# BolinLai/CSTS

Hardware: AMD Instinct MI355X
Metric: clips/sec training (fwd+bwd) CSTS-Ego4D 16x256^2 bf16 (higher is better)
Workload: dtype bf16; 1 GPU; CSTS_Ego4D_Gaze_Forecast.yaml train step (fwd + KLDiv + 0.05*EgoNCE + bwd + clip + AdamW), 16x256^2 video + 24 kHz STFT audio, b=4/GPU; mode=train, global_batch=4, frames=16, crop=256, parallelism=dp1, step=hip_graph, hip_graph=True, rccl_ranks=1

## Files before the change

### csts_amd/csrc/attention.hip

```cpp
#include <type_traits>
#include <utility>
#include "common.h"

#ifndef CSTS_ATTN_PART
#define CSTS_ATTN_PART 0
#endif
#ifndef CSTS_DKV_DEPTH
#define CSTS_DKV_DEPTH 4
#endif
#ifndef CSTS_DKV_SWZ
#define CSTS_DKV_SWZ 0
#endif

#ifdef CSTS_ATTN_STAMPS
#if CSTS_ATTN_PART == 1
__device__ unsigned long long g_attn_stamps[4096];
#else
static __device__ unsigned long long g_attn_stamps[4096];
#endif
#define AT_STAMP() do { if (stamp_on && nstamp < 4000) g_attn_stamps[nstamp++] = (unsigned long long)__builtin_amdgcn_s_memtime(); } while (0)
#if CSTS_ATTN_PART == 1
extern "C" int csts_debug_attn_stamps(unsigned long long* dst_host) {
  return (int)hipMemcpyFromSymbol(dst_host, HIP_SYMBOL(g_attn_stamps), sizeof(unsigned long long) * 4096);
}
// ... 1465 lines not shown
  CSTS_REQUIRE(a->O && a->LSE && aligned16(a->O) && strides_ok(a->o_strides, a->dtype), "bad output");
  AttnP p; fill(a, p);
  dim3 grid((unsigned)cdiv(a->Nq, 128), a->H, a->B);
  CSTS_REQUIRE(attn_dispatch(K_FWD, a, p, grid, stream), "hipFuncSetAttribute(MaxDynamicSharedMemorySize) failed on this device");
  CSTS_LAUNCH_CHECK();
  return 0;
}

extern "C" size_t csts_attn_bwd_workspace(const csts_attn_args* a) {
  if (!a) return 0;
  int nsplit, q_chunk;
  dkv_plan(a, nsplit, q_chunk);
  return nsplit > 1 ? (size_t)2 * nsplit * a->B * a->H * a->Nk * a->head_dim * sizeof(float) : 16;
}

extern "C" int csts_attn_bwd(const csts_attn_args* a, void* workspace, size_t ws_bytes, hipStream_t stream) {
  ATTN_COMMON_CHECKS(a);
  CSTS_REQUIRE(a->O && a->LSE && a->dO && a->delta && a->dQ && a->dK && a->dV, "null backward operand");
  CSTS_REQUIRE(aligned16(a->dO) && aligned16(a->dQ) && aligned16(a->dK) && aligned16(a->dV), "alignment");
  CSTS_REQUIRE(strides_ok(a->do_strides, a->dtype) && strides_ok(a->dq_strides, a->dtype) &&
                   strides_ok(a->dk_strides, a->dtype) && strides_ok(a->dv_strides, a->dtype) &&
                   strides_ok(a->o_strides, a->dtype), "strides must keep 16-byte row alignment");
  AttnP p; fill(a, p);
  if (fused_bwd_ok(a)) {
    dkv_plan(a, p.nsplit, p.q_chunk);
    if (p.nsplit > 1) {
      CSTS_REQUIRE(workspace != nullptr && ws_bytes >= csts_attn_bwd_workspace(a), "workspace too small");
      p.ws = reinterpret_cast<float*>(workspace);
    }
    hipLaunchKernelGGL((attn_bwd_fused_kernel<96>), dim3((unsigned)p.nsplit, (unsigned)(a->B * a->H)), dim3(256), 0, stream, p);
    CSTS_LAUNCH_CHECK();
    if (p.nsplit > 1) {
      const int64_t total = (int64_t)2 * a->B * a->H * a->Nk * a->head_dim / 8;
      hipLaunchKernelGGL(attn_dkv_reduce_kernel, dim3((unsigned)std::min<int64_t>(cdiv(total, 256), 4096)), dim3(256), 0,
                         stream, p, a->head_dim);
      CSTS_LAUNCH_CHECK();
    }
    return 0;
  }
  {
    dim3 grid((unsigned)cdiv(a->Nq, 128), a->H, a->B);
    CSTS_REQUIRE(attn_dispatch(K_DQ, a, p, grid, stream), "hipFuncSetAttribute(MaxDynamicSharedMemorySize) failed on this device");
    CSTS_LAUNCH_CHECK();
  }
  {
    dkv_plan(a, p.nsplit, p.q_chunk);
    if (p.nsplit > 1) {
      CSTS_REQUIRE(workspace != nullptr && ws_bytes >= csts_attn_bwd_workspace(a), "workspace too small");
      p.ws = reinterpret_cast<float*>(workspace);
    }
    dim3 grid((unsigned)cdiv(a->Nk, 128), p.nsplit, a->B * a->H);
    CSTS_REQUIRE(attn_dispatch(K_DKV, a, p, grid, stream), "hipFuncSetAttribute(MaxDynamicSharedMemorySize) failed on this device");
    CSTS_LAUNCH_CHECK();
    if (p.nsplit > 1) {
      const int64_t total = (int64_t)2 * a->B * a->H * a->Nk * a->head_dim / 8;
      hipLaunchKernelGGL(attn_dkv_reduce_kernel, dim3((unsigned)std::min<int64_t>(cdiv(total, 256), 4096)), dim3(256), 0,
                         stream, p, a->head_dim);
      CSTS_LAUNCH_CHECK();
    }
  }
  return 0;
}

extern "C" int csts_attn_probs(const csts_attn_args* a, float* probs, hipStream_t stream) {
  ATTN_COMMON_CHECKS(a);
  CSTS_REQUIRE(a->LSE && probs, "null pointer");
  AttnP p; fill(a, p);
  const int64_t total = (int64_t)a->B * a->H * a->Nq * a->Nk;
  hipLaunchKernelGGL(attn_probs_kernel, dim3((unsigned)std::min<int64_t>(cdiv(total, 256), 4096)), dim3(256), 0, stream, p,
                     a->head_dim, probs);
  CSTS_LAUNCH_CHECK();
  return 0;
}
#else
}
bool csts_attn_dkv_fast_launch(const csts_attn::AttnP& p, dim3 grid, hipStream_t stream) {
// ... 7 lines not shown
```

### csts_amd/csrc/common.h

```cpp
#pragma once
#include <hip/hip_runtime.h>
#include <stdint.h>
#include <stddef.h>
#include <string>

#include "../../include/csts_hip.h"

#ifdef CSTS_HALF_F16
typedef _Float16 bf16;
typedef _Float16 bf16x8 __attribute__((ext_vector_type(8)));
typedef _Float16 bf16x4 __attribute__((ext_vector_type(4)));
typedef _Float16 bf16x2 __attribute__((ext_vector_type(2)));
#define CSTS_MFMA16 __builtin_amdgcn_mfma_f32_32x32x16_f16
#else
typedef __bf16 bf16;
typedef __bf16 bf16x8 __attribute__((ext_vector_type(8)));
typedef __bf16 bf16x4 __attribute__((ext_vector_type(4)));
typedef __bf16 bf16x2 __attribute__((ext_vector_type(2)));
#define CSTS_MFMA16 __builtin_amdgcn_mfma_f32_32x32x16_bf16
#endif
typedef short s16x4 __attribute__((ext_vector_type(4)));
typedef float f32x16 __attribute__((ext_vector_type(16)));
typedef float f32x4 __attribute__((ext_vector_type(4)));
typedef float f32x2 __attribute__((ext_vector_type(2)));
// ... 149 lines not shown
}
__device__ __forceinline__ float gelu_fast(float x) {
  const float t = x * 0.70710678118654752f, ax = fabsf(t);
  const float e = __expf(-ax * ax);
  const float er = copysignf(erf_poly_times_exp(ax, e), x);
  return 0.5f * x * (1.0f + er);
}
__device__ __forceinline__ float dgelu_fast(float x) {
  const float t = x * 0.70710678118654752f, ax = fabsf(t);
  const float e = __expf(-ax * ax);
  const float er = copysignf(erf_poly_times_exp(ax, e), x);
  return 0.5f * (1.0f + er) + x * 0.39894228040143268f * e;
}

int csts_reduce_rows_launch(const float* ws, float* out, int64_t nrows, int64_t ncols, float scale, hipStream_t s);
```

### csts_amd/csrc/norm.hip

```cpp
#include "common.h"

namespace {

constexpr int MAXV = 12;
constexpr int LN_BWD_WAVES = 8;

template <bool F32> __device__ __forceinline__ float ldt(const void* p, int64_t i) {
  if constexpr (F32) return reinterpret_cast<const float*>(p)[i];
  else return h16_lo((unsigned)reinterpret_cast<const unsigned short*>(p)[i]);
}
template <bool F32> __device__ __forceinline__ void stt(void* p, int64_t i, float v) {
  if constexpr (F32) reinterpret_cast<float*>(p)[i] = v;
  else reinterpret_cast<bf16*>(p)[i] = (bf16)v;
}

struct FwdAdd {
  const void* addend = nullptr;
  void* sum = nullptr;
};
template <int NV, int R, bool XF32, bool YF32>
__global__ __launch_bounds__(256) void ln_fwd_kernel(const void* __restrict__ x, const float* __restrict__ gamma,
                                                     const float* __restrict__ beta, void* __restrict__ y,
                                                     float* __restrict__ mean, float* __restrict__ rstd, int64_t rows,
                                                     int C, float eps, FwdAdd fa) {
// ... 252 lines not shown
        if (sub == 0) {
          if (mean) mean[row] = mu;
          if (rstd) rstd[row] = rs;
        }
      }
    }
  }
}

#ifndef CSTS_LN_BWD_R
#define CSTS_LN_BWD_R 1
#endif
#ifndef CSTS_LN_BWD_MINW
#define CSTS_LN_BWD_MINW 1
#endif
template <int GL, int NCH, int R, bool DYF32, bool XF32>
__global__ __launch_bounds__(512, CSTS_LN_BWD_MINW) void ln_bwd_vec_kernel(const void* __restrict__ dy, const void* __restrict__ x,
                                                         const float* __restrict__ gamma, const float* __restrict__ mean,
                                                         const float* __restrict__ rstd, void* __restrict__ dx,
                                                         const void* __restrict__ addend, float* __restrict__ ws, int64_t rows,
                                                         int C, const float* __restrict__ gamma1, Copy16 dx16) {
  extern __shared__ __attribute__((aligned(16))) float red[];
  const int64_t ro = (int64_t)blockIdx.y * rows;
  if (blockIdx.y == 1) gamma = gamma1;
  ws += (int64_t)blockIdx.y * gridDim.x * 2 * C;
  const int sub = threadIdx.x % GL, gib = threadIdx.x / GL;
  constexpr int GPB = 512 / GL;
  const int64_t grp = xcd_block(blockIdx.x, gridDim.x) * GPB + gib, ngrp = (int64_t)gridDim.x * GPB;
  int c0[NCH];
  bool act[NCH];
  float gm[NCH][8], dg[NCH][8], db[NCH][8];
#pragma unroll
  for (int i = 0; i < NCH; ++i) {
    const int c = (sub + GL * i) * 8;
    act[i] = c < C;
    c0[i] = min(c, C - 8);
    ld8t<true>(gamma, c0[i], gm[i]);
#pragma unroll
    for (int j = 0; j < 8; ++j) { dg[i][j] = 0.f; db[i][j] = 0.f; }
  }
  const float invC = 1.f / C;
  for (int64_t row0 = grp * R; row0 < rows; row0 += ngrp * R) {
    float d[R][NCH][8], xv[R][NCH][8], ad[R][NCH][8], mu[R], rs[R];
#pragma unroll
    for (int r = 0; r < R; ++r) {
      const int64_t row = ro + min(row0 + r, rows - 1);
      mu[r] = mean[row];
      rs[r] = rstd[row];
#pragma unroll
      for (int i = 0; i < NCH; ++i) {
        ld8t<DYF32>(dy, row * C + c0[i], d[r][i]);
        if (dx16.dy2) {
          float d2[8];
          ld8t<DYF32>(dx16.dy2, row * C + c0[i], d2);
#pragma unroll
          for (int j = 0; j < 8; ++j) d[r][i][j] += d2[j];
        }
        ld8t<XF32>(x, row * C + c0[i], xv[r][i]);
        if (addend) ld8t<XF32>(addend, row * C + c0[i], ad[r][i]);
        else {
#pragma unroll
          for (int j = 0; j < 8; ++j) ad[r][i][j] = 0.f;
        }
      }
    }
#pragma unroll
// ... 181 lines not shown
  else if (xf) hipLaunchKernelGGL((ln_bwd_kernel<NV, R, false, true>), grid, dim3(64 * LN_BWD_WAVES), sh, st, dy, x, g, mean, rstd, dx, addend, ws, rows, C, g1, dx16);
  else hipLaunchKernelGGL((ln_bwd_kernel<NV, R, false, false>), grid, dim3(64 * LN_BWD_WAVES), sh, st, dy, x, g, mean, rstd, dx, addend, ws, rows, C, g1, dx16);
}
template <int GL, int NCH, int R>
static void ln_fwd_vec_launch(bool xf, bool yf, dim3 grid, hipStream_t st, const void* x, const float* g, const float* b, void* y,
                              float* mean, float* rstd, int64_t rows, int C, float eps, FwdAdd fa) {
  if (xf && yf) hipLaunchKernelGGL((ln_fwd_vec_kernel<GL, NCH, R, true, true>), grid, dim3(256), 0, st, x, g, b, y, mean, rstd, rows, C, eps, fa);
  else if (xf) hipLaunchKernelGGL((ln_fwd_vec_kernel<GL, NCH, R, true, false>), grid, dim3(256), 0, st, x, g, b, y, mean, rstd, rows, C, eps, fa);
  else if (yf) hipLaunchKernelGGL((ln_fwd_vec_kernel<GL, NCH, R, false, true>), grid, dim3(256), 0, st, x, g, b, y, mean, rstd, rows, C, eps, fa);
  else hipLaunchKernelGGL((ln_fwd_vec_kernel<GL, NCH, R, false, false>), grid, dim3(256), 0, st, x, g, b, y, mean, rstd, rows, C, eps, fa);
}
template <int GL, int NCH, int R>
static void ln_bwd_vec_launch(bool df, bool xf, dim3 grid, size_t sh, hipStream_t st, const void* dy, const void* x, const float* g,
                              const float* mean, const float* rstd, void* dx, const void* addend, float* ws, int64_t rows, int C,
                              const float* g1, Copy16 dx16) {
  if (df && xf) hipLaunchKernelGGL((ln_bwd_vec_kernel<GL, NCH, R, true, true>), grid, dim3(512), sh, st, dy, x, g, mean, rstd, dx, addend, ws, rows, C, g1, dx16);
  else if (df) hipLaunchKernelGGL((ln_bwd_vec_kernel<GL, NCH, R, true, false>), grid, dim3(512), sh, st, dy, x, g, mean, rstd, dx, addend, ws, rows, C, g1, dx16);
  else if (xf) hipLaunchKernelGGL((ln_bwd_vec_kernel<GL, NCH, R, false, true>), grid, dim3(512), sh, st, dy, x, g, mean, rstd, dx, addend, ws, rows, C, g1, dx16);
  else hipLaunchKernelGGL((ln_bwd_vec_kernel<GL, NCH, R, false, false>), grid, dim3(512), sh, st, dy, x, g, mean, rstd, dx, addend, ws, rows, C, g1, dx16);
}
static bool ln_vec_ok(int C, std::initializer_list<const void*> ptrs) {
  if (C % 8 != 0 || C < 8 || C > 1024) return false;
  for (const void* q : ptrs)
    if (q != nullptr && !aligned16(q)) return false;
  return true;
}
static int ln_group_lanes(int C) { return C <= 128 ? 16 : (C <= 256 ? 32 : 64); }
#ifndef CSTS_LN_FWD_R
#define CSTS_LN_FWD_R 2
#endif
static int64_t ln_fwd_vec_blocks(int64_t rows, int C) { return std::min<int64_t>(cdiv(rows * ln_group_lanes(C), 256 * (C <= 512 ? CSTS_LN_FWD_R : 2)), 4096); }
static bool ln_bwd_vec(bool df, bool xf, dim3 grid, hipStream_t st, const void* dy, const void* x, const float* g, const float* mean,
                       const float* rstd, void* dx, const void* addend, float* ws, int64_t rows, int C, const float* g1, Copy16 dx16) {
  const size_t sh = (size_t)(512 / ln_group_lanes(C)) * 2 * C * sizeof(float);
// ... 120 lines not shown
    }
    return 0;
  }
  if (C <= 128) ln_bwd_launch<2, 4>(df, xf, grid, sh, stream, dy, x, gamma0, mean, rstd, dx, nullptr, ws, rows, C, gamma1);
  else if (C <= 192) ln_bwd_launch<3, 4>(df, xf, grid, sh, stream, dy, x, gamma0, mean, rstd, dx, nullptr, ws, rows, C, gamma1);
  else if (C <= 384) ln_bwd_launch<6, 2>(df, xf, grid, sh, stream, dy, x, gamma0, mean, rstd, dx, nullptr, ws, rows, C, gamma1);
  else ln_bwd_launch<12, 1>(df, xf, grid, sh, stream, dy, x, gamma0, mean, rstd, dx, nullptr, ws, rows, C, gamma1);
  CSTS_LAUNCH_CHECK();
  if (dgb0 != nullptr) {
    csts_reduce_rows_launch(ws, dgb0, nb, 2 * C, 1.f, stream);
    csts_reduce_rows_launch(ws + nb * 2 * C, dgb1, nb, 2 * C, 1.f, stream);
    CSTS_LAUNCH_CHECK();
  }
  return 0;
}
```

### csts_amd/csrc/stencil.hip

```cpp
#include "common.h"
#include <algorithm>
#include <cstdlib>
#include <cstring>
#include <vector>

namespace {

struct Geom {
  int B, C, HD;
  int Tf, Hf, Wf;
  int Tc, Hc, Wc;
  int st, sh, sw;
  int64_t f_bs, f_ts;
  int64_t c_bs, c_ts;
};

constexpr int VEC = 4;

__device__ __forceinline__ void ld4(const void* p, int dt, int64_t i, float (&o)[4]) {
  if (dt == CSTS_F32) {
    float4 a = *reinterpret_cast<const float4*>(reinterpret_cast<const float*>(p) + i);
    o[0] = a.x; o[1] = a.y; o[2] = a.z; o[3] = a.w;
  } else {
    bf16x4 a = *reinterpret_cast<const bf16x4*>(reinterpret_cast<const bf16*>(p) + i);
// ... 25 lines not shown
  return dt == CSTS_F32 ? (const void*)(reinterpret_cast<const float*>(p) + off) : (const void*)(reinterpret_cast<const bf16*>(p) + off);
}
__device__ __forceinline__ void* batch_ptr(void* p, int dt, int64_t off) {
  return dt == CSTS_F32 ? (void*)(reinterpret_cast<float*>(p) + off) : (void*)(reinterpret_cast<bf16*>(p) + off);
}

__device__ __forceinline__ void stage_weights(const float* __restrict__ w, float* wl, int HD) {
  const int nthr = blockDim.x * blockDim.y, tid = threadIdx.y * blockDim.x + threadIdx.x;
  for (int i = tid; i < HD * 27; i += nthr) {
    const int k = i / HD, c = i - k * HD;
    wl[i] = w[c * 27 + k];
  }
  __syncthreads();
}

struct FastDiv { unsigned m; int sh; int d; };
__device__ __forceinline__ int fdiv(int n, const FastDiv& f) { return (int)(((unsigned long long)(unsigned)n * f.m) >> f.sh); }
struct RowGeom {
  Geom g;
  int lt, lh, lw;
  FastDiv dNc, dHc, dWc;
  FastDiv dNf, dHf, dWf;
  FastDiv dN2, dH2, dW2;
  FastDiv dC4, dC8, dHD, dHeads;
};
__device__ __forceinline__ void decompf(int bt, const FastDiv& dN, const FastDiv& dH, const FastDiv& dW, int& b, int& t, int& h, int& w) {
  b = fdiv(bt, dN);
  int o = bt - b * dN.d;
  const int q = fdiv(o, dW);
  w = o - q * dW.d;
  t = fdiv(q, dH);
  h = q - t * dH.d;
// ... 1069 lines not shown
  return on;
}
bool fast_row(int row_tokens, int C, int64_t rows, FastRow& fr) {
  fr.cq = C / VEC;
  fr.wq = row_tokens * fr.cq;
  fr.inv_cq = 1.f / (float)fr.cq;
  return resample_fast_on() && C % VEC == 0 && fr.cq <= 256 && fr.wq <= 16384 && rows <= 65535 * (int64_t)1 && rows > 0;
}

int grid_for(int64_t total) { return (int)std::min<int64_t>(cdiv(total, 256), 256 * 32); }
int grid_for_staged(int64_t total) { return (int)std::min<int64_t>(cdiv(total, 256), 256 * 4); }

int ilog2(int v) { if (v <= 0 || (v & (v - 1)) != 0) return -1; int l = 0; while ((1 << l) < v) ++l; return l; }
bool pow2(int v) { return v > 0 && (v & (v - 1)) == 0; }

FastDiv fast_div(int d) {
  FastDiv f; f.d = d;
  if (d <= 1) { f.m = 1; f.sh = 0; return f; }
  int sft = 0;
  while ((1LL << sft) < d) ++sft;
  const unsigned long long num = 1ULL << (31 + sft);
  f.m = (unsigned)((num + d - 1) / d);
  f.sh = 31 + sft;
  return f;
}
int fill_geom(const csts_dwconv_geom* a, RowGeom& rg) {
  Geom& g = rg.g;
  g.B = a->B; g.C = a->C; g.HD = a->HD;
  g.Tf = a->Tf; g.Hf = a->Hf; g.Wf = a->Wf; g.Tc = a->Tc; g.Hc = a->Hc; g.Wc = a->Wc;
  g.st = a->st; g.sh = a->sh; g.sw = a->sw;
  g.f_bs = a->fine_batch_stride; g.f_ts = a->fine_token_stride;
  g.c_bs = a->coarse_batch_stride; g.c_ts = a->coarse_token_stride;
  rg.lt = ilog2(a->st); rg.lh = ilog2(a->sh); rg.lw = ilog2(a->sw);
  rg.dNc = fast_div(a->Tc * a->Hc * a->Wc); rg.dHc = fast_div(a->Hc); rg.dWc = fast_div(a->Wc);
  rg.dNf = fast_div(a->Tf * a->Hf * a->Wf); rg.dHf = fast_div(a->Hf); rg.dWf = fast_div(a->Wf);
  rg.dN2 = fast_div(std::max(1, a->Tf * (a->Hf / 2) * (a->Wf / 2))); rg.dH2 = fast_div(std::max(1, a->Hf / 2)); rg.dW2 = fast_div(std::max(1, a->Wf / 2));
  rg.dC4 = fast_div(std::max(1, a->C / 4)); rg.dC8 = fast_div(std::max(1, a->C / 8)); rg.dHD = fast_div(a->HD); rg.dHeads = fast_div(a->C / a->HD);
  return 0;
}

// ... 353 lines not shown
```

### csts_amd/lib.py

```python
from __future__ import annotations

import ctypes as C
import os

_lib = None


class CstsError(RuntimeError):
    pass


_HERE = os.path.dirname(os.path.abspath(__file__))
LIB_PATH = os.environ.get("CSTS_HIP_LIB") or os.path.join(_HERE, "libcsts_hip.so")
HALF = os.environ.get("CSTS_HALF", "bf16")
_PATHS = {"bf16": LIB_PATH, "fp16": os.environ.get("CSTS_HIP_LIB_F16") or os.path.join(_HERE, "libcsts_hip_f16.so")}


def set_half(kind: str):
    global HALF, LIB_PATH
    if kind not in _PATHS:
        raise ValueError(f"16-bit type must be 'bf16' or 'fp16', got {kind!r}")
    if _lib is not None and kind != HALF:
        raise CstsError(f"this process already runs the {HALF} kernel library; the {kind} build is a different shared object "
                        "(one 16-bit activation type per process: start a new process for the other mode)")
    HALF = kind
    LIB_PATH = _PATHS[kind]


def half_dtype():
    import torch
    return torch.float16 if HALF == "fp16" else torch.bfloat16


ABI_VERSION = 11
F32, BF16 = 0, 1
GEMM_NT, GEMM_NN, GEMM_TN = 0, 1, 2
EPI_NONE, EPI_GELU, EPI_DGELU = 0, 1, 2
MASK_NONE, MASK_SPATIAL = 0, 1
GAZE_DECODE_MAX_HW = 8192
AUDIO_PIXEL_MAX_SIDE, AUDIO_PIXEL_MAX_HW = 128, 4096

vp = C.c_void_p
i64 = C.c_int64
sz = C.c_size_t


class GemmArgs(C.Structure):
    _fields_ = [("layout", C.c_int),
                ("A", vp), ("a_dt", C.c_int), ("lda", i64),
# ... 36 lines not shown
    _fields_ = [("B", C.c_int), ("C", C.c_int),
                ("Ti", C.c_int), ("Hi", C.c_int), ("Wi", C.c_int),
                ("To", C.c_int), ("Ho", C.c_int), ("Wo", C.c_int),
                ("st", C.c_int), ("sh", C.c_int), ("sw", C.c_int)]


class AttnArgs(C.Structure):
    _fields_ = [("Q", vp), ("K", vp), ("V", vp), ("O", vp), ("LSE", vp),
                ("dO", vp), ("delta", vp), ("dQ", vp), ("dK", vp), ("dV", vp),
                ("dtype", C.c_int), ("B", C.c_int), ("H", C.c_int), ("Nq", C.c_int), ("Nk", C.c_int),
                ("head_dim", C.c_int),
                ("q_strides", i64 * 3), ("k_strides", i64 * 3), ("v_strides", i64 * 3), ("o_strides", i64 * 3),
                ("do_strides", i64 * 3), ("dq_strides", i64 * 3), ("dk_strides", i64 * 3), ("dv_strides", i64 * 3),
                ("scale", C.c_float),
                ("mask_mode", C.c_int), ("mask_T", C.c_int), ("mask_HW", C.c_int)]


class Im2colGeom(C.Structure):
    _fields_ = [("B", C.c_int), ("Cin", C.c_int), ("T", C.c_int), ("H", C.c_int), ("W", C.c_int),
                ("kernel", C.c_int * 3), ("stride", C.c_int * 3), ("padding", C.c_int * 3),
                ("To", C.c_int), ("Ho", C.c_int), ("Wo", C.c_int), ("Kpad", C.c_int)]


class TokenSegment(C.Structure):
    _fields_ = [("src", vp), ("dst", vp), ("src_bs", i64), ("dst_bs", i64), ("src_off", i64), ("dst_off", i64), ("n", C.c_int), ("pad_", C.c_int)]


class KvRowsGeom(C.Structure):
    _fields_ = [("B", C.c_int), ("C", C.c_int), ("T", C.c_int), ("H", C.c_int), ("W", C.c_int), ("sh", C.c_int), ("sw", C.c_int),
                ("Hc", C.c_int), ("Wc", C.c_int)]
# ... 66 lines not shown
    "csts_dwconv_wgrad_workspace": (sz, [C.POINTER(DwconvGeom)]),
    "csts_dwconv_wgrad": (_I, [C.POINTER(DwconvGeom), vp, _I, vp, _I, vp, vp, sz, vp]),
    "csts_dwconv_transposed2": (_I, [C.POINTER(DwconvGeom), vp * 2, _I, vp * 2, vp * 2, _I, vp]),
    "csts_dwconv_wgrad2": (_I, [C.POINTER(DwconvGeom), vp * 2, _I, vp * 2, _I, vp * 2, vp, sz, vp]),
    "csts_dwconv_wgrad_grouped_workspace": (sz, [C.POINTER(DwconvGeom)]),
    "csts_dwconv_wgrad_grouped_plan": (_I, [C.POINTER(DwconvWgradItem), _I, vp, sz, C.POINTER(C.c_int)]),
    "csts_dwconv_wgrad_grouped": (_I, [vp, _I, _I, _I, vp]),
    "csts_pool_ln_fwd": (_I, [C.POINTER(PoolLnArgs), vp]),
    "csts_maxpool_fwd": (_I, [C.POINTER(PoolGeom), vp, _I, vp, vp, vp]),
    "csts_maxpool_bwd": (_I, [C.POINTER(PoolGeom), vp, _I, vp, vp, vp]),
    "csts_trilinear_fwd": (_I, [C.POINTER(PoolGeom), vp, _I, vp, _I, vp, _I, vp]),
    "csts_trilinear_bwd": (_I, [C.POINTER(PoolGeom), vp, _I, vp, _I, vp]),
    "csts_attn_fwd": (_I, [C.POINTER(AttnArgs), vp]),
    "csts_attn_bwd_workspace": (sz, [C.POINTER(AttnArgs)]),
    "csts_attn_bwd": (_I, [C.POINTER(AttnArgs), vp, sz, vp]),
    "csts_attn_probs": (_I, [C.POINTER(AttnArgs), vp, vp]),
    "csts_im2col": (_I, [C.POINTER(Im2colGeom), vp, _I, vp, _I, vp]),
    "csts_posembed_build": (_I, [vp, vp, vp, _I, _I, _I, vp]),
    "csts_transpose_batched": (_I, [vp, _I, vp, _I, i64, _I, _I, vp]),
    "csts_transpose_multi": (_I, [vp, _I, vp]),
    "csts_colsum_workspace": (sz, [i64, i64, i64]),
    "csts_colsum": (_I, [vp, _I, vp, vp, i64, i64, i64, vp, sz, vp]),
    "csts_axpby": (_I, [vp, _I, vp, _I, vp, _I, i64, _F, _F, vp]),
    "csts_rows_gather": (_I, [C.POINTER(KvRowsGeom), vp, _I, vp, vp]),
    "csts_copy_token_segments": (_I, [C.POINTER(TokenSegment), _I, _I, _I, _I, vp]),
    "csts_rows_scatter_add": (_I, [C.POINTER(KvRowsGeom), vp, _I, vp, _I, vp]),
    "csts_scale_rows": (_I, [vp, _I, vp, i64, vp, _I, i64, i64, vp]),
    "csts_dropout_fwd": (_I, [vp, vp, vp, i64, vp, _I, vp, _U32, _U32, _F, i64, i64, vp]),
    "csts_dropout_bwd": (_I, [vp, _I, vp, i64, vp, _I, vp, _U32, _U32, _F, i64, i64, vp]),
    "csts_dropout_mask": (_I, [vp, _U32, _U32, vp, i64, vp]),
# ... 88 lines not shown
```

### csts_amd/ops.py

```python
from __future__ import annotations

import collections
import contextlib
import ctypes as C
import functools
import math
import os
import weakref
from typing import Optional, Sequence, Tuple

import torch
from torch.autograd import Function

from . import lib as L

F32, BF16 = L.F32, L.BF16


def _lib():
    return L.load()


def _dt(t: torch.Tensor) -> int:
    if t.dtype == torch.float32:
# ... 1158 lines not shown
        QW = Cc if kvc is not None else 3 * Cc
        if kvc is not None:
            dkvc = torch.empty_like(kvc)
            kv_fine, kv_dfine, kv_off = kvc, dkvc, (0, Cc)
        else:
            dkvc, kv_fine, kv_dfine, kv_off = None, qkv, dqkv, (Cc, 2 * Cc)
        delta = torch.empty(B, H, Nq, dtype=torch.float32, device=dev)

        def grad_target(slot, n_rows):
            if slot in saved:
                t = torch.empty(B, n_rows, Cc, dtype=qkv.dtype, device=dev)
                return t, 0, (n_rows * Cc, Cc, HD)
            return dqkv, slot * Cc, (N * QW, QW, HD)

        tq = grad_target(0, Nq)
        if "kv" in saved:
            dkv = torch.empty(2, B, Nk, Cc, dtype=qkv.dtype, device=dev)
            tk, tv = (dkv[0], 0, (Nk * Cc, Cc, HD)), (dkv[1], 0, (Nk * Cc, Cc, HD))
        else:
            tk, tv = grad_target(1, Nk), grad_target(2, Nk)
        a = L.AttnArgs()
        a.Q, a.K, a.V = _p(qd[0], qd[1]), _p(kd[0], kd[1]), _p(vd[0], vd[1])
        a.O, a.LSE, a.dO, a.delta = _p(o), _p(lse), _p(do), _p(delta)
        a.dQ, a.dK, a.dV = _p(tq[0], tq[1]), _p(tk[0], tk[1]), _p(tv[0], tv[1])
        a.dtype, a.B, a.H, a.Nq, a.Nk, a.head_dim = _dt(qkv), B, H, Nq, Nk, HD
        a.q_strides = (C.c_int64 * 3)(*qd[2])
        a.k_strides = (C.c_int64 * 3)(*kd[2])
        a.v_strides = (C.c_int64 * 3)(*vd[2])
        a.o_strides = (C.c_int64 * 3)(Nq * Cc, Cc, HD)
        a.do_strides = (C.c_int64 * 3)(Nq * Cc, Cc, HD)
        a.dq_strides = (C.c_int64 * 3)(*tq[2])
        a.dk_strides = (C.c_int64 * 3)(*tk[2])
        a.dv_strides = (C.c_int64 * 3)(*tv[2])
        a.scale = HD ** -0.5
        a.mask_mode, a.mask_T, a.mask_HW = mask_mode, mask_T, mask_HW
        ws = _ws(lib.csts_attn_bwd_workspace(C.byref(a)), dev)
        L.check(lib.csts_attn_bwd(C.byref(a), _p(ws), ws.numel(), s), "csts_attn_bwd")

        grads = {}

        P = ctx.params

        def pooled_bwd(slot, dy, w, gamma, transposed):
            c, mean, rstd, g = saved[slot]
            pw, pg, pb = P[3 * slot], P[3 * slot + 1], P[3 * slot + 2]
            dc, dg, db = _ln_rows_bwd(dy, c, gamma, mean, rstd, HD, params=(pg, pb))
            defer = _can_defer(pw)
            grouped = defer and _stencil_group_now()
            wsz = (lib.csts_dwconv_wgrad_grouped_workspace if grouped else lib.csts_dwconv_wgrad_workspace)(C.byref(g))
            wws = _ws(wsz, dev)
            dw = torch.empty(HD * 27, dtype=torch.float32, device=dev)
            dwp = None if defer else _p(dw)
            if grouped:
                if transposed:
                    _queue_stencil_wgrad(g, dc, 0, qkv, slot * Cc, wws)
                else:
# ... 8 lines not shown
                L.check(lib.csts_dwconv_strided(C.byref(g), _p(dc), _dt(dc), _p(w), _p(dqkv, slot * Cc), _dt(dqkv), s),
                        "csts_dwconv_strided(bwd)")
            else:
                L.check(lib.csts_dwconv_transposed(C.byref(g), _p(dc), _dt(dc), _p(w), _p(dqkv, slot * Cc), _dt(dqkv), s),
                        "csts_dwconv_transposed(bwd)")
            dwv = dw.view(HD, 1, 3, 3, 3)
            if defer:
                _defer(wws, dw, wsz // (HD * 27 * 4), HD * 27)
                _assign_later(pw, dwv)
                dwv = None
            grads[slot] = (dwv, dg, db)

        def pooled_bwd_kv():
            c2, mean2, rstd2, g = saved["kv"]
            rows = B * Nk * H
            dc2 = torch.empty_like(c2)
            dgb = torch.empty(2, 2 * HD, dtype=torch.float32, device=dev)
            nbytes = lib.csts_layernorm_bwd_workspace(rows, HD)
            lws = _ws(2 * nbytes, dev)
            defer = _can_defer(P[3], P[4], P[5], P[6], P[7], P[8])
            L.check(lib.csts_layernorm_bwd2(_p(dkv), _dt(dkv), _p(c2), _dt(c2), _p(gk), _p(gv), _p(mean2), _p(rstd2), _p(dc2),
                                            _dt(dc2), None if defer else _p(dgb[0]), None if defer else _p(dgb[1]), _p(lws),
                                            lws.numel(), rows, HD, s), "csts_layernorm_bwd2")
            if defer:
                nrow = nbytes // (2 * HD * 4)
                _defer(lws[:nbytes], dgb[0], nrow, 2 * HD)
                _defer(lws[nbytes:], dgb[1], nrow, 2 * HD)
            vp2 = C.c_void_p * 2
            L.check(lib.csts_dwconv_transposed2(C.byref(g), vp2(_p(dc2[0]), _p(dc2[1])), _dt(dc2), vp2(_p(wk), _p(wv)),
                                                vp2(_p(kv_dfine, kv_off[0]), _p(kv_dfine, kv_off[1])), _dt(kv_dfine), s),
                    "csts_dwconv_transposed2")
            grouped = defer and _stencil_group_now()
            wsz = (lib.csts_dwconv_wgrad_grouped_workspace if grouped else lib.csts_dwconv_wgrad_workspace)(C.byref(g))
            wws = _ws(2 * wsz, dev)
            dw = torch.empty(2, HD * 27, dtype=torch.float32, device=dev)
            dwp = vp2(None, None) if defer else vp2(_p(dw[0]), _p(dw[1]))
            if grouped:
                for i in (0, 1):
# ... 19 lines not shown
        if "kv" in saved:
            pooled_bwd_kv()
        elif 1 in saved:
            pooled_bwd(1, tk[0], wk, gk, False)
            pooled_bwd(2, tv[0], wv, gv, False)
        gq_ = grads.get(0, (None, None, None))
        gk_ = grads.get(1, (None, None, None))
        gv_ = grads.get(2, (None, None, None))
        return (dqkv, dkvc, gq_[0], gq_[1], gq_[2], gk_[0], gk_[1], gk_[2], gv_[0], gv_[1], gv_[2], None)


def attention_inner(qkv, wq, gq, bq, wk, gk, bk, wv, gv, bv, meta, kvc=None):
    return AttnInnerFn.apply(qkv, kvc, wq, gq, bq, wk, gk, bk, wv, gv, bv, meta)


KV_COMPACT_MIN_STRIDE = int(os.environ.get("CSTS_KV_COMPACT", "8"))


def kv_compact_dims(thw, stride_kv):
    out = []
    for n, st in zip(thw[1:], stride_kv[1:]):
        no = (n - 1) // st + 1
        out.append(3 * no - 1 - (1 if (no - 1) * st + 1 > n - 1 else 0))
    return tuple(out)


def kv_compact_ok(thw, stride_kv, has_pool_kv) -> bool:
    return bool(has_pool_kv and KV_COMPACT_MIN_STRIDE > 0 and stride_kv[0] == 1 and stride_kv[1] >= max(3, KV_COMPACT_MIN_STRIDE)
                and stride_kv[2] >= max(3, KV_COMPACT_MIN_STRIDE))

# ... 1022 lines not shown
```

### include/csts_hip.h

```cpp
#ifndef CSTS_HIP_H
#define CSTS_HIP_H

#include <stddef.h>
#include <stdint.h>

#ifdef __cplusplus
extern "C" {
#endif

#ifndef __HIP_PLATFORM_AMD__
typedef struct ihipStream_t* hipStream_t;
#endif

enum { CSTS_F32 = 0, CSTS_BF16 = 1, CSTS_HALF = 1 };
enum { CSTS_GEMM_NT = 0, CSTS_GEMM_NN = 1, CSTS_GEMM_TN = 2 };
enum { CSTS_EPI_NONE = 0, CSTS_EPI_GELU = 1, CSTS_EPI_DGELU = 2 };
enum { CSTS_MASK_NONE = 0, CSTS_MASK_SPATIAL = 1 };

#define CSTS_ABI_VERSION 11
const char* csts_last_error(void);
int csts_abi_version(void);
int csts_half_kind(void);

typedef struct {
  int layout;
  const void* A; int a_dt; int64_t lda;
  const void* B; int b_dt; int64_t ldb;
  void* C; int c_dt; int64_t ldc;
  int64_t M, N, K;
  const float* bias;
  int epilogue;
  void* aux; int aux_dt; int64_t ldaux;
  const void* residual; int r_dt; int64_t ldr; int64_t res_row_mod;
  const float* row_scale; int64_t rows_per_scale;
// ... 92 lines not shown
                       int y_dt, hipStream_t stream);
int csts_trilinear_bwd(const csts_pool_geom* g, const void* dy, int dy_dt, void* dx, int dx_dt, hipStream_t stream);

typedef struct {
  const void* Q; const void* K; const void* V; void* O; float* LSE;
  const void* dO; float* delta; void* dQ; void* dK; void* dV;
  int dtype, B, H, Nq, Nk, head_dim;
  int64_t q_strides[3], k_strides[3], v_strides[3], o_strides[3];
  int64_t do_strides[3], dq_strides[3], dk_strides[3], dv_strides[3];
  float scale;
  int mask_mode, mask_T, mask_HW;
} csts_attn_args;
int csts_attn_fwd(const csts_attn_args* a, hipStream_t stream);
size_t csts_attn_bwd_workspace(const csts_attn_args* a);
int csts_attn_bwd(const csts_attn_args* a, void* workspace, size_t ws_bytes, hipStream_t stream);
int csts_attn_probs(const csts_attn_args* a, float* probs , hipStream_t stream);

typedef struct {
  int B, Cin, T, H, W;
  int kernel[3], stride[3], padding[3];
  int To, Ho, Wo;
  int Kpad;
} csts_im2col_geom;
int csts_im2col(const csts_im2col_geom* g, const void* x, int x_dt, void* col, int col_dt, hipStream_t stream);
int csts_posembed_build(const float* spatial, const float* temporal, float* pos, int T, int HW, int C, hipStream_t stream);

int csts_transpose_batched(const void* in, int in_dt, void* out, int out_dt, int64_t batch, int R, int Cc,
                           hipStream_t stream);
typedef struct { const void* src; void* dst; int R, C, r0, c0; } csts_transpose_tile;
int csts_transpose_multi(const csts_transpose_tile* device_tiles, int ntiles, hipStream_t stream);
// ... 175 lines not shown
```

Baseline: 200.5 clips/s.

## Fuse split-K dK/dV reduction into the pooled KV LayerNorm backward

When the attention backward splits queries and writes fp32 partial dK/dV slabs, the KV LayerNorm backward now sums those slabs directly instead of running a separate reduce kernel that writes a bf16 dkv tensor which the LayerNorm then reads back. This removes one kernel launch and a full round trip of the dK/dV tensor through memory. The LayerNorm kernel gains a SPLIT template path that remaps rows across the slab layout with fast division and rounds the sum to bf16 to match the old numerics. It is on by default through an environment flag and falls back to the old path when alignment or the split plan do not allow it.

```diff
diff --git a/csts_amd/csrc/attention.hip b/csts_amd/csrc/attention.hip
--- a/csts_amd/csrc/attention.hip
+++ b/csts_amd/csrc/attention.hip
@@ -1503,14 +1503,29 @@
   return nsplit > 1 ? (size_t)2 * nsplit * a->B * a->H * a->Nk * a->head_dim * sizeof(float) : 16;
 }
 
-extern "C" int csts_attn_bwd(const csts_attn_args* a, void* workspace, size_t ws_bytes, hipStream_t stream) {
+static int kvln_tail(const csts_attn_args* a, const csts_attn_kvln_args* t, const AttnP& p, hipStream_t stream) {
+  return csts_ln_bwd2_split_launch(p.ws, p.nsplit, a->B, a->H, a->Nk, t->c2, a->dtype, t->gamma_k, t->gamma_v, t->mean, t->rstd, t->dc2,
+                                   t->dgb0, t->dgb1, t->ln_workspace, t->ln_ws_bytes, a->head_dim, stream);
+}
+
+static int attn_bwd_run(const csts_attn_args* a, const csts_attn_kvln_args* tail, void* workspace, size_t ws_bytes, hipStream_t stream) {
   ATTN_COMMON_CHECKS(a);
-  CSTS_REQUIRE(a->O && a->LSE && a->dO && a->delta && a->dQ && a->dK && a->dV, "null backward operand");
-  CSTS_REQUIRE(aligned16(a->dO) && aligned16(a->dQ) && aligned16(a->dK) && aligned16(a->dV), "alignment");
+  CSTS_REQUIRE(a->O && a->LSE && a->dO && a->delta && a->dQ && (tail || (a->dK && a->dV)), "null backward operand");
+  CSTS_REQUIRE(aligned16(a->dO) && aligned16(a->dQ) && (tail || (aligned16(a->dK) && aligned16(a->dV))), "alignment");
   CSTS_REQUIRE(strides_ok(a->do_strides, a->dtype) && strides_ok(a->dq_strides, a->dtype) &&
-                   strides_ok(a->dk_strides, a->dtype) && strides_ok(a->dv_strides, a->dtype) &&
+                   (tail || (strides_ok(a->dk_strides, a->dtype) && strides_ok(a->dv_strides, a->dtype))) &&
                    strides_ok(a->o_strides, a->dtype), "strides must keep 16-byte row alignment");
   AttnP p; fill(a, p);
+  if (tail) {
+    dkv_plan(a, p.nsplit, p.q_chunk);
+    CSTS_REQUIRE(p.nsplit > 1, "the plan does not split the queries: call csts_attn_bwd and csts_layernorm_bwd2");
+    CSTS_REQUIRE(tail->c2 && tail->gamma_k && tail->gamma_v && tail->mean && tail->rstd && tail->dc2 && tail->ln_workspace, "null LayerNorm operand");
+    CSTS_REQUIRE((tail->dgb0 == nullptr) == (tail->dgb1 == nullptr), "dgb0/dgb1: both or neither (neither = deferred second stage)");
+    CSTS_REQUIRE(workspace != nullptr && ws_bytes >= csts_attn_bwd_workspace(a), "workspace too small");
+    CSTS_REQUIRE(csts_ln_bwd2_split_ok(reinterpret_cast<const float*>(workspace), tail->c2, tail->gamma_k, tail->gamma_v, tail->dc2, a->B,
+                                       a->H, a->Nk, a->head_dim), "the vector LayerNorm backward needs 16-byte aligned operands");
+    CSTS_REQUIRE(tail->ln_ws_bytes >= 2 * csts_layernorm_bwd_workspace((int64_t)a->B * a->Nk * a->H, a->head_dim), "LayerNorm workspace too small");
+  }
   if (fused_bwd_ok(a)) {
     dkv_plan(a, p.nsplit, p.q_chunk);
     if (p.nsplit > 1) {
@@ -1519,6 +1534,7 @@
     }
     hipLaunchKernelGGL((attn_bwd_fused_kernel<96>), dim3((unsigned)p.nsplit, (unsigned)(a->B * a->H)), dim3(256), 0, stream, p);
     CSTS_LAUNCH_CHECK();
+    if (tail) return kvln_tail(a, tail, p, stream);
     if (p.nsplit > 1) {
       const int64_t total = (int64_t)2 * a->B * a->H * a->Nk * a->head_dim / 8;
       hipLaunchKernelGGL(attn_dkv_reduce_kernel, dim3((unsigned)std::min<int64_t>(cdiv(total, 256), 4096)), dim3(256), 0,
@@ -1541,6 +1557,7 @@
     dim3 grid((unsigned)cdiv(a->Nk, 128), p.nsplit, a->B * a->H);
     CSTS_REQUIRE(attn_dispatch(K_DKV, a, p, grid, stream), "hipFuncSetAttribute(MaxDynamicSharedMemorySize) failed on this device");
     CSTS_LAUNCH_CHECK();
+    if (tail) return kvln_tail(a, tail, p, stream);
     if (p.nsplit > 1) {
       const int64_t total = (int64_t)2 * a->B * a->H * a->Nk * a->head_dim / 8;
       hipLaunchKernelGGL(attn_dkv_reduce_kernel, dim3((unsigned)std::min<int64_t>(cdiv(total, 256), 4096)), dim3(256), 0,
@@ -1549,6 +1566,16 @@
     }
   }
   return 0;
+}
+
+extern "C" int csts_attn_bwd(const csts_attn_args* a, void* workspace, size_t ws_bytes, hipStream_t stream) {
+  return attn_bwd_run(a, nullptr, workspace, ws_bytes, stream);
+}
+
+extern "C" int csts_attn_bwd_kvln(const csts_attn_args* a, const csts_attn_kvln_args* t, void* workspace, size_t ws_bytes,
+                                  hipStream_t stream) {
+  CSTS_REQUIRE(t != nullptr, "null LayerNorm arguments");
+  return attn_bwd_run(a, t, workspace, ws_bytes, stream);
 }
 
 extern "C" int csts_attn_probs(const csts_attn_args* a, float* probs, hipStream_t stream) {
diff --git a/csts_amd/csrc/common.h b/csts_amd/csrc/common.h
--- a/csts_amd/csrc/common.h
+++ b/csts_amd/csrc/common.h
@@ -187,3 +187,32 @@
 }
 
 int csts_reduce_rows_launch(const float* ws, float* out, int64_t nrows, int64_t ncols, float scale, hipStream_t s);
+
+struct FastDiv { unsigned m; int sh; int d; };
+__host__ __device__ __forceinline__ int fdiv(int n, const FastDiv& f) { return (int)(((unsigned long long)(unsigned)n * f.m) >> f.sh); }
+static inline FastDiv fast_div(int d) {
+  FastDiv f; f.d = d;
+  if (d <= 1) { f.m = 1; f.sh = 0; return f; }
+  int sft = 0;
+  while ((1LL << sft) < d) ++sft;
+  const unsigned long long num = 1ULL << (31 + sft);
+  f.m = (unsigned)((num + d - 1) / d);
+  f.sh = 31 + sft;
+  return f;
+}
+
+struct KvSlab { FastDiv dH, dNk; int hd; int64_t per; };
+static inline KvSlab kv_slab(int B, int H, int Nk, int hd) {
+  KvSlab s; s.dH = fast_div(H); s.dNk = fast_div(Nk); s.hd = hd; s.per = (int64_t)B * H * Nk * hd;
+  return s;
+}
+__host__ __device__ __forceinline__ int64_t kv_slab_row(const KvSlab& s, int row) {
+  const int t = fdiv(row, s.dH), head = row - t * s.dH.d;
+  const int b = fdiv(t, s.dNk), k = t - b * s.dNk.d;
+  return ((int64_t)(b * s.dH.d + head) * s.dNk.d + k) * s.hd;
+}
+bool csts_ln_bwd2_split_ok(const float* slabs, const void* x, const float* gamma0, const float* gamma1, void* dx, int B, int H, int Nk,
+                           int C);
+int csts_ln_bwd2_split_launch(const float* slabs, int nsplit, int B, int H, int Nk, const void* x, int x_dt, const float* gamma0,
+                              const float* gamma1, const float* mean, const float* rstd, void* dx, float* dgb0, float* dgb1,
+                              void* workspace, size_t ws_bytes, int C, hipStream_t stream);
diff --git a/csts_amd/csrc/norm.hip b/csts_amd/csrc/norm.hip
--- a/csts_amd/csrc/norm.hip
+++ b/csts_amd/csrc/norm.hip
@@ -290,12 +290,17 @@
 #ifndef CSTS_LN_BWD_MINW
 #define CSTS_LN_BWD_MINW 1
 #endif
-template <int GL, int NCH, int R, bool DYF32, bool XF32>
+struct SplitSrc {
+  const float* ws = nullptr;
+  int nsplit = 0;
+  KvSlab slab;
+};
+template <int GL, int NCH, int R, bool DYF32, bool XF32, bool SPLIT = false>
 __global__ __launch_bounds__(512, CSTS_LN_BWD_MINW) void ln_bwd_vec_kernel(const void* __restrict__ dy, const void* __restrict__ x,
                                                          const float* __restrict__ gamma, const float* __restrict__ mean,
                                                          const float* __restrict__ rstd, void* __restrict__ dx,
                                                          const void* __restrict__ addend, float* __restrict__ ws, int64_t rows,
-                                                         int C, const float* __restrict__ gamma1, Copy16 dx16) {
+                                                         int C, const float* __restrict__ gamma1, Copy16 dx16, SplitSrc ss) {
   extern __shared__ __attribute__((aligned(16))) float red[];
   const int64_t ro = (int64_t)blockIdx.y * rows;
   if (blockIdx.y == 1) gamma = gamma1;
@@ -323,9 +328,28 @@
       const int64_t row = ro + min(row0 + r, rows - 1);
       mu[r] = mean[row];
       rs[r] = rstd[row];
+      const float* part = nullptr;
+      if constexpr (SPLIT)
+        part = ss.ws + (int64_t)blockIdx.y * ss.nsplit * ss.slab.per + kv_slab_row(ss.slab, (int)(row - ro));
 #pragma unroll
       for (int i = 0; i < NCH; ++i) {
-        ld8t<DYF32>(dy, row * C + c0[i], d[r][i]);
+        if constexpr (SPLIT) {
+          float t[8];
+#pragma unroll
+          for (int j = 0; j < 8; ++j) d[r][i][j] = 0.f;
+#pragma unroll 4
+          for (int sp = 0; sp < ss.nsplit; ++sp) {
+            ld8t<true>(part, sp * ss.slab.per + c0[i], t);
+#pragma unroll
+            for (int j = 0; j < 8; ++j) d[r][i][j] += t[j];
+          }
+          if constexpr (!XF32) {
+#pragma unroll
+            for (int j = 0; j < 8; ++j) d[r][i][j] = (float)(bf16)d[r][i][j];
+          }
+        } else {
+          ld8t<DYF32>(dy, row * C + c0[i], d[r][i]);
+        }
         if (dx16.dy2) {
           float d2[8];
           ld8t<DYF32>(dx16.dy2, row * C + c0[i], d2);
@@ -537,10 +561,16 @@
 static void ln_bwd_vec_launch(bool df, bool xf, dim3 grid, size_t sh, hipStream_t st, const void* dy, const void* x, const float* g,
                               const float* mean, const float* rstd, void* dx, const void* addend, float* ws, int64_t rows, int C,
                               const float* g1, Copy16 dx16) {
-  if (df && xf) hipLaunchKernelGGL((ln_bwd_vec_kernel<GL, NCH, R, true, true>), grid, dim3(512), sh, st, dy, x, g, mean, rstd, dx, addend, ws, rows, C, g1, dx16);
-  else if (df) hipLaunchKernelGGL((ln_bwd_vec_kernel<GL, NCH, R, true, false>), grid, dim3(512), sh, st, dy, x, g, mean, rstd, dx, addend, ws, rows, C, g1, dx16);
-  else if (xf) hipLaunchKernelGGL((ln_bwd_vec_kernel<GL, NCH, R, false, true>), grid, dim3(512), sh, st, dy, x, g, mean, rstd, dx, addend, ws, rows, C, g1, dx16);
-  else hipLaunchKernelGGL((ln_bwd_vec_kernel<GL, NCH, R, false, false>), grid, dim3(512), sh, st, dy, x, g, mean, rstd, dx, addend, ws, rows, C, g1, dx16);
+  if (df && xf) hipLaunchKernelGGL((ln_bwd_vec_kernel<GL, NCH, R, true, true>), grid, dim3(512), sh, st, dy, x, g, mean, rstd, dx, addend, ws, rows, C, g1, dx16, SplitSrc{});
+  else if (df) hipLaunchKernelGGL((ln_bwd_vec_kernel<GL, NCH, R, true, false>), grid, dim3(512), sh, st, dy, x, g, mean, rstd, dx, addend, ws, rows, C, g1, dx16, SplitSrc{});
+  else if (xf) hipLaunchKernelGGL((ln_bwd_vec_kernel<GL, NCH, R, false, true>), grid, dim3(512), sh, st, dy, x, g, mean, rstd, dx, addend, ws, rows, C, g1, dx16, SplitSrc{});
+  else hipLaunchKernelGGL((ln_bwd_vec_kernel<GL, NCH, R, false, false>), grid, dim3(512), sh, st, dy, x, g, mean, rstd, dx, addend, ws, rows, C, g1, dx16, SplitSrc{});
+}
+template <int GL>
+static void ln_bwd_vec_split_launch(bool xf, dim3 grid, size_t sh, hipStream_t st, const SplitSrc& ss, const void* x, const float* g,
+                                    const float* mean, const float* rstd, void* dx, float* ws, int64_t rows, int C, const float* g1) {
+  if (xf) hipLaunchKernelGGL((ln_bwd_vec_kernel<GL, 1, CSTS_LN_BWD_R, true, true, true>), grid, dim3(512), sh, st, nullptr, x, g, mean, rstd, dx, nullptr, ws, rows, C, g1, Copy16{}, ss);
+  else hipLaunchKernelGGL((ln_bwd_vec_kernel<GL, 1, CSTS_LN_BWD_R, false, false, true>), grid, dim3(512), sh, st, nullptr, x, g, mean, rstd, dx, nullptr, ws, rows, C, g1, Copy16{}, ss);
 }
 static bool ln_vec_ok(int C, std::initializer_list<const void*> ptrs) {
   if (C % 8 != 0 || C < 8 || C > 1024) return false;
@@ -691,3 +721,37 @@
   }
   return 0;
 }
+
+bool csts_ln_bwd2_split_ok(const float* slabs, const void* x, const float* gamma0, const float* gamma1, void* dx, int B, int H, int Nk,
+                           int C) {
+  const int64_t rows = (int64_t)B * Nk * H;
+  return (C == 96 || C == 192) && rows > 0 && rows * C < (1LL << 31) && ln_vec_ok(C, {slabs, x, dx, gamma0, gamma1}) &&
+         (rows * C) % 8 == 0 && (size_t)(512 / ln_group_lanes(C)) * 2 * C * sizeof(float) <= 65536;
+}
+int csts_ln_bwd2_split_launch(const float* slabs, int nsplit, int B, int H, int Nk, const void* x, int x_dt, const float* gamma0,
+                              const float* gamma1, const float* mean, const float* rstd, void* dx, float* dgb0, float* dgb1,
+                              void* workspace, size_t ws_bytes, int C, hipStream_t stream) {
+  CSTS_REQUIRE(slabs && x && gamma0 && gamma1 && mean && rstd && dx && workspace, "null pointer");
+  CSTS_REQUIRE(nsplit > 1, "the split-sum form is for split plans");
+  CSTS_REQUIRE((dgb0 == nullptr) == (dgb1 == nullptr), "dgb0/dgb1: both or neither (neither = deferred second stage)");
+  CSTS_REQUIRE(csts_ln_bwd2_split_ok(slabs, x, gamma0, gamma1, dx, B, H, Nk, C),
+               "needs head_dim 96 or 192, 16-byte aligned operands and fewer than 2^31 elements per tensor");
+  const int64_t rows = (int64_t)B * Nk * H;
+  const int64_t nb = ln_bwd_blocks(rows, C);
+  CSTS_REQUIRE(ws_bytes >= (size_t)2 * nb * 2 * C * sizeof(float), "workspace too small");
+  const dim3 grid((unsigned)nb, 2);
+  const size_t sh = (size_t)(512 / ln_group_lanes(C)) * 2 * C * sizeof(float);
+  float* ws = reinterpret_cast<float*>(workspace);
+  SplitSrc ss;
+  ss.ws = slabs; ss.nsplit = nsplit; ss.slab = kv_slab(B, H, Nk, C);
+  const bool xf = x_dt == CSTS_F32;
+  if (C <= 128) ln_bwd_vec_split_launch<16>(xf, grid, sh, stream, ss, x, gamma0, mean, rstd, dx, ws, rows, C, gamma1);
+  else ln_bwd_vec_split_launch<32>(xf, grid, sh, stream, ss, x, gamma0, mean, rstd, dx, ws, rows, C, gamma1);
+  CSTS_LAUNCH_CHECK();
+  if (dgb0 != nullptr) {
+    csts_reduce_rows_launch(ws, dgb0, nb, 2 * C, 1.f, stream);
+    csts_reduce_rows_launch(ws + nb * 2 * C, dgb1, nb, 2 * C, 1.f, stream);
+    CSTS_LAUNCH_CHECK();
+  }
+  return 0;
+}
diff --git a/csts_amd/csrc/stencil.hip b/csts_amd/csrc/stencil.hip
--- a/csts_amd/csrc/stencil.hip
+++ b/csts_amd/csrc/stencil.hip
@@ -63,8 +63,6 @@
   __syncthreads();
 }
 
-struct FastDiv { unsigned m; int sh; int d; };
-__device__ __forceinline__ int fdiv(int n, const FastDiv& f) { return (int)(((unsigned long long)(unsigned)n * f.m) >> f.sh); }
 struct RowGeom {
   Geom g;
   int lt, lh, lw;
@@ -1164,16 +1162,6 @@
 int ilog2(int v) { if (v <= 0 || (v & (v - 1)) != 0) return -1; int l = 0; while ((1 << l) < v) ++l; return l; }
 bool pow2(int v) { return v > 0 && (v & (v - 1)) == 0; }
 
-FastDiv fast_div(int d) {
-  FastDiv f; f.d = d;
-  if (d <= 1) { f.m = 1; f.sh = 0; return f; }
-  int sft = 0;
-  while ((1LL << sft) < d) ++sft;
-  const unsigned long long num = 1ULL << (31 + sft);
-  f.m = (unsigned)((num + d - 1) / d);
-  f.sh = 31 + sft;
-  return f;
-}
 int fill_geom(const csts_dwconv_geom* a, RowGeom& rg) {
   Geom& g = rg.g;
   g.B = a->B; g.C = a->C; g.HD = a->HD;
diff --git a/csts_amd/lib.py b/csts_amd/lib.py
--- a/csts_amd/lib.py
+++ b/csts_amd/lib.py
@@ -32,7 +32,7 @@
     return torch.float16 if HALF == "fp16" else torch.bfloat16
 
 
-ABI_VERSION = 11
+ABI_VERSION = 12
 F32, BF16 = 0, 1
 GEMM_NT, GEMM_NN, GEMM_TN = 0, 1, 2
 EPI_NONE, EPI_GELU, EPI_DGELU = 0, 1, 2
@@ -99,6 +99,11 @@
                 ("do_strides", i64 * 3), ("dq_strides", i64 * 3), ("dk_strides", i64 * 3), ("dv_strides", i64 * 3),
                 ("scale", C.c_float),
                 ("mask_mode", C.c_int), ("mask_T", C.c_int), ("mask_HW", C.c_int)]
+
+
+class AttnKvlnArgs(C.Structure):
+    _fields_ = [("c2", vp), ("gamma_k", vp), ("gamma_v", vp), ("mean", vp), ("rstd", vp), ("dc2", vp),
+                ("dgb0", vp), ("dgb1", vp), ("ln_workspace", vp), ("ln_ws_bytes", sz)]
 
 
 class Im2colGeom(C.Structure):
@@ -195,6 +200,7 @@
     "csts_attn_fwd": (_I, [C.POINTER(AttnArgs), vp]),
     "csts_attn_bwd_workspace": (sz, [C.POINTER(AttnArgs)]),
     "csts_attn_bwd": (_I, [C.POINTER(AttnArgs), vp, sz, vp]),
+    "csts_attn_bwd_kvln": (_I, [C.POINTER(AttnArgs), C.POINTER(AttnKvlnArgs), vp, sz, vp]),
     "csts_attn_probs": (_I, [C.POINTER(AttnArgs), vp, vp]),
     "csts_im2col": (_I, [C.POINTER(Im2colGeom), vp, _I, vp, _I, vp]),
     "csts_posembed_build": (_I, [vp, vp, vp, _I, _I, _I, vp]),
diff --git a/csts_amd/ops.py b/csts_amd/ops.py
--- a/csts_amd/ops.py
+++ b/csts_amd/ops.py
@@ -1196,16 +1196,22 @@
             return dqkv, slot * Cc, (N * QW, QW, HD)
 
         tq = grad_target(0, Nq)
-        if "kv" in saved:
+        a = L.AttnArgs()
+        a.Q, a.K, a.V = _p(qd[0], qd[1]), _p(kd[0], kd[1]), _p(vd[0], vd[1])
+        a.dtype, a.B, a.H, a.Nq, a.Nk, a.head_dim = _dt(qkv), B, H, Nq, Nk, HD
+        a.mask_mode, a.mask_T, a.mask_HW = mask_mode, mask_T, mask_HW
+        ws_bytes = lib.csts_attn_bwd_workspace(C.byref(a))
+        kvln = bool(ATTN_KVLN and "kv" in saved and ws_bytes > 16 and HD % 8 == 0 and saved["kv"][0].data_ptr() % 16 == 0
+                    and gk.data_ptr() % 16 == 0 and gv.data_ptr() % 16 == 0)
+        if kvln:
+            tk = tv = (None, 0, (Nk * Cc, Cc, HD))
+        elif "kv" in saved:
             dkv = torch.empty(2, B, Nk, Cc, dtype=qkv.dtype, device=dev)
             tk, tv = (dkv[0], 0, (Nk * Cc, Cc, HD)), (dkv[1], 0, (Nk * Cc, Cc, HD))
         else:
             tk, tv = grad_target(1, Nk), grad_target(2, Nk)
-        a = L.AttnArgs()
-        a.Q, a.K, a.V = _p(qd[0], qd[1]), _p(kd[0], kd[1]), _p(vd[0], vd[1])
         a.O, a.LSE, a.dO, a.delta = _p(o), _p(lse), _p(do), _p(delta)
         a.dQ, a.dK, a.dV = _p(tq[0], tq[1]), _p(tk[0], tk[1]), _p(tv[0], tv[1])
-        a.dtype, a.B, a.H, a.Nq, a.Nk, a.head_dim = _dt(qkv), B, H, Nq, Nk, HD
         a.q_strides = (C.c_int64 * 3)(*qd[2])
         a.k_strides = (C.c_int64 * 3)(*kd[2])
         a.v_strides = (C.c_int64 * 3)(*vd[2])
@@ -1215,13 +1221,23 @@
         a.dk_strides = (C.c_int64 * 3)(*tk[2])
         a.dv_strides = (C.c_int64 * 3)(*tv[2])
         a.scale = HD ** -0.5
-        a.mask_mode, a.mask_T, a.mask_HW = mask_mode, mask_T, mask_HW
-        ws = _ws(lib.csts_attn_bwd_workspace(C.byref(a)), dev)
-        L.check(lib.csts_attn_bwd(C.byref(a), _p(ws), ws.numel(), s), "csts_attn_bwd")
+        ws = _ws(ws_bytes, dev)
+        P = ctx.params
+        if kvln:
+            c2, mean2, rstd2, _g = saved["kv"]
+            kv_dc2 = torch.empty_like(c2)
+            kv_dgb = torch.empty(2, 2 * HD, dtype=torch.float32, device=dev)
+            kv_lws = _ws(2 * lib.csts_layernorm_bwd_workspace(B * Nk * H, HD), dev)
+            kv_defer = _can_defer(P[3], P[4], P[5], P[6], P[7], P[8])
+            t = L.AttnKvlnArgs()
+            t.c2, t.gamma_k, t.gamma_v, t.mean, t.rstd, t.dc2 = _p(c2), _p(gk), _p(gv), _p(mean2), _p(rstd2), _p(kv_dc2)
+            t.dgb0, t.dgb1 = (None, None) if kv_defer else (_p(kv_dgb[0]), _p(kv_dgb[1]))
+            t.ln_workspace, t.ln_ws_bytes = _p(kv_lws), kv_lws.numel()
+            L.check(lib.csts_attn_bwd_kvln(C.byref(a), C.byref(t), _p(ws), ws.numel(), s), "csts_attn_bwd_kvln")
+        else:
+            L.check(lib.csts_attn_bwd(C.byref(a), _p(ws), ws.numel(), s), "csts_attn_bwd")
 
         grads = {}
-
-        P = ctx.params
 
         def pooled_bwd(slot, dy, w, gamma, transposed):
             c, mean, rstd, g = saved[slot]
@@ -1260,14 +1276,17 @@
         def pooled_bwd_kv():
             c2, mean2, rstd2, g = saved["kv"]
             rows = B * Nk * H
-            dc2 = torch.empty_like(c2)
-            dgb = torch.empty(2, 2 * HD, dtype=torch.float32, device=dev)
             nbytes = lib.csts_layernorm_bwd_workspace(rows, HD)
-            lws = _ws(2 * nbytes, dev)
-            defer = _can_defer(P[3], P[4], P[5], P[6], P[7], P[8])
-            L.check(lib.csts_layernorm_bwd2(_p(dkv), _dt(dkv), _p(c2), _dt(c2), _p(gk), _p(gv), _p(mean2), _p(rstd2), _p(dc2),
-                                            _dt(dc2), None if defer else _p(dgb[0]), None if defer else _p(dgb[1]), _p(lws),
-                                            lws.numel(), rows, HD, s), "csts_layernorm_bwd2")
+            if kvln:
+                dc2, dgb, lws, defer = kv_dc2, kv_dgb, kv_lws, kv_defer
+            else:
+                dc2 = torch.empty_like(c2)
+                dgb = torch.empty(2, 2 * HD, dtype=torch.float32, device=dev)
+                lws = _ws(2 * nbytes, dev)
+                defer = _can_defer(P[3], P[4], P[5], P[6], P[7], P[8])
+                L.check(lib.csts_layernorm_bwd2(_p(dkv), _dt(dkv), _p(c2), _dt(c2), _p(gk), _p(gv), _p(mean2), _p(rstd2), _p(dc2),
+                                                _dt(dc2), None if defer else _p(dgb[0]), None if defer else _p(dgb[1]), _p(lws),
+                                                lws.numel(), rows, HD, s), "csts_layernorm_bwd2")
             if defer:
                 nrow = nbytes // (2 * HD * 4)
                 _defer(lws[:nbytes], dgb[0], nrow, 2 * HD)
@@ -1317,6 +1336,7 @@
     return AttnInnerFn.apply(qkv, kvc, wq, gq, bq, wk, gk, bk, wv, gv, bv, meta)
 
 
+ATTN_KVLN = os.environ.get("CSTS_ATTN_KVLN", "1") != "0"
 KV_COMPACT_MIN_STRIDE = int(os.environ.get("CSTS_KV_COMPACT", "8"))
 
 
diff --git a/include/csts_hip.h b/include/csts_hip.h
--- a/include/csts_hip.h
+++ b/include/csts_hip.h
@@ -17,7 +17,7 @@
 enum { CSTS_EPI_NONE = 0, CSTS_EPI_GELU = 1, CSTS_EPI_DGELU = 2 };
 enum { CSTS_MASK_NONE = 0, CSTS_MASK_SPATIAL = 1 };
 
-#define CSTS_ABI_VERSION 11
+#define CSTS_ABI_VERSION 12
 const char* csts_last_error(void);
 int csts_abi_version(void);
 int csts_half_kind(void);
@@ -140,6 +140,15 @@
 int csts_attn_fwd(const csts_attn_args* a, hipStream_t stream);
 size_t csts_attn_bwd_workspace(const csts_attn_args* a);
 int csts_attn_bwd(const csts_attn_args* a, void* workspace, size_t ws_bytes, hipStream_t stream);
+typedef struct {
+  const void* c2;
+  const float* gamma_k; const float* gamma_v;
+  const float* mean; const float* rstd;
+  void* dc2;
+  float* dgb0; float* dgb1;
+  void* ln_workspace; size_t ln_ws_bytes;
+} csts_attn_kvln_args;
+int csts_attn_bwd_kvln(const csts_attn_args* a, const csts_attn_kvln_args* t, void* workspace, size_t ws_bytes, hipStream_t stream);
 int csts_attn_probs(const csts_attn_args* a, float* probs , hipStream_t stream);
 
 typedef struct {
```

Result: no change. 201.5 clips/s, median of 6 (+0.5%).
